# danielecook/seq-collection

Measured on AMD Instinct MI355X. Metric: Gbases/s parsed (fq-count), higher is better.
Workload: dtype u8; 1 GPU; synthetic 10 GB uncompressed 150 bp Illumina FASTQ per GPU, HBM-resident (BASELINE configs[1]; the N>1 lines of this bench hold 25 GB per GPU — `--bytes-per-gpu 25e9` at N=1 is their like-for-like anchor); bytes_per_gpu=10000000326, seed=20260101, exchange=none, flags=0

## Files before the change

seq-collection_amd/csrc/fq_scan_kernels.hpp:

```cpp
#pragma once
#include <hip/hip_runtime.h>
#include <stdint.h>

#include "scfq_hdrhash.hpp"

#ifndef SCFQ_ABLATE
#define SCFQ_ABLATE 0
#endif

namespace scfq {

constexpr int kTile = 4096;
constexpr int kWavesPerBlock = 4;
constexpr int kRing = 2;
constexpr int kPartialWords = 32;
constexpr uint32_t kMaxTilesPerRange = 960;

enum : int { W_NL = 0, W_GC = 1, W_N = 5, W_LEN = 9, W_STARTS = 13, W_FAT = 17, W_FPLUS = 21, W_BYTES = 25, W_LAST = 26 };

constexpr uint32_t F_QUAL_HIST = 1u, F_STRUCT = 2u;

constexpr int kHistRep = 4;
constexpr int kHistWords = 256 * 4 * kHistRep;
constexpr int kHistWaves = 2;
// ... 683 lines not shown
    }
    const uint32_t shl = (sh0 + cnt * 8u) & 31u;
    t_len += (64u - cnt - s_len) << shl;
    t_gc += (64u - popc64(WGC) - s_gc) << shl;
    t_nn += (64u - popc64(WNN) - s_nn) << shl;
  }

  st.p_len = t_len; st.p_gc = t_gc; st.p_nn = t_nn; st.p_crlf = t_crlf;
  if (STRUCT) { st.p_fat = t_fat; st.p_fpl = t_fpl; }
  if (++st.pending == 3) flush_pending(st);
  st.phase = (st.phase + total) & 3u;
  st.nl_total += total;
  st.prev_last = (int32_t)((uint32_t)__builtin_amdgcn_readlane((int)d[15], 63) >> 24);
}

struct ScanArgs {
  const uint8_t* base;
  uint64_t n;
  int32_t prev_byte;
  uint32_t tiles_per_range;
  uint64_t n_ranges;
  uint64_t* partials;
  uint32_t* hist_partials;
  const uint8_t* todo;
  const uint8_t* guess;
  uint32_t* hist_wg;
  uint8_t* guess_out;
  uint32_t guess_cap_tiles;
};

template <bool STRUCT, int HIST, int RING = kRing, bool NT = true, bool GUESS = false>
__global__ __launch_bounds__(HIST == 1 ? 64 * kHistWaves : HIST == 2 ? 64 * kQWaves : 64 * kWavesPerBlock, (HIST == 2 && !GUESS) ? SCFQ_QOCC : 1) void fq_scan_tiles(ScanArgs a) {
  constexpr int WAVES = HIST == 1 ? kHistWaves : HIST == 2 ? kQWaves : kWavesPerBlock;
  static_assert(RING >= 2 && RING <= 4, "ring depth");
  static_assert(!GUESS || (STRUCT && HIST == 0), "the guess pass is the K4 accounting without partials");
  extern __shared__ __attribute__((aligned(16))) uint8_t smem[];
  const int lane = threadIdx.x & 63;
  const uint32_t wave = (uint32_t)__builtin_amdgcn_readfirstlane((int)(threadIdx.x >> 6));
  uint8_t* ring = smem + (HIST == 2 ? kQWords * 4 : 0) + wave * (RING * kTile);
  const uint64_t range = (uint64_t)blockIdx.x * WAVES + wave;
  bool active = range < a.n_ranges;
  if (HIST == 1 && active && a.todo) active = (a.todo[range] != 0);
  if (HIST != 2 && !active) return;
  uint32_t* hist_lds = nullptr;
  if (HIST == 1) {
    hist_lds = reinterpret_cast<uint32_t*>(smem + WAVES * RING * kTile) + wave * kHistWords;
    for (int k = lane; k < kHistWords; k += 64) hist_lds[k] = 0;
  }
  if (HIST == 2) {
    hist_lds = reinterpret_cast<uint32_t*>(smem);
    if ((uint32_t)(uintptr_t)hist_lds & (kQWords * 4 - 1)) __builtin_trap();
    for (int k = threadIdx.x; k < kQWords; k += 64 * WAVES) hist_lds[k] = 0;
    __syncthreads();
  }
  if (active) {

  const uint64_t B = (uint64_t)(uintptr_t)a.base, E = B + a.n;
  const uint64_t A0 = B & ~(uint64_t)(kTile - 1);
// ... 96 lines not shown
      }
    }
  }
  if (GUESS) {
    if (lane == 0) a.guess_out[range] = (uint8_t)guessed;
    return;
  }

  flush_pending(st);
  uint64_t* out = a.partials + range * kPartialWords;
  auto sum4 = [&](const Acc16& acc) {
    const uint32_t c0 = wave_sum(acc.e & 0xFFFFu), c2 = wave_sum(acc.e >> 16);
    const uint32_t c1 = wave_sum(acc.o & 0xFFFFu), c3 = wave_sum(acc.o >> 16);
    return make_uint4(c0, c1, c2, c3);
  };
  auto store4 = [&](int w, uint64_t v0, uint64_t v1, uint64_t v2, uint64_t v3) {
    if (lane == 0) { out[w + 0] = v0; out[w + 1] = v1; out[w + 2] = v2; out[w + 3] = v3; }
  };
  const uint4 gc4 = sum4(st.gc), nn4 = sum4(st.nn), len4 = sum4(st.len), cr4 = sum4(st.crlf);
  store4(W_GC, gc4.x, gc4.y, gc4.z, gc4.w);
  store4(W_N, nn4.x, nn4.y, nn4.z, nn4.w);
  store4(W_LEN, (uint64_t)len4.x - cr4.x, (uint64_t)len4.y - cr4.y, (uint64_t)len4.z - cr4.z, (uint64_t)len4.w - cr4.w);
  if (STRUCT) {
    const uint4 a4 = sum4(st.fat), p4 = sum4(st.fplus);
    const uint64_t last_at = ((A0 + (uint64_t)t_end * kTile < E) ? A0 + (uint64_t)t_end * kTile : E) - 1;
    const uint32_t last_is_nl = (*reinterpret_cast<const uint8_t*>(last_at) == (uint8_t)'\n') ? 1u : 0u;
    const uint32_t nfol = st.nl_total - last_is_nl;
    const uint32_t first_is_start = (range_prev == '\n' || range_prev == -1) ? 1u : 0u;
    const uint4 s4 = make_uint4((nfol >> 2) + first_is_start, (nfol + 3u) >> 2, (nfol + 2u) >> 2, (nfol + 1u) >> 2);
    store4(W_STARTS, s4.x, s4.y, s4.z, s4.w);
    store4(W_FAT, a4.x, a4.y, a4.z, a4.w);
    store4(W_FPLUS, p4.x, p4.y, p4.z, p4.w);
  } else {
    store4(W_STARTS, 0, 0, 0, 0); store4(W_FAT, 0, 0, 0, 0); store4(W_FPLUS, 0, 0, 0, 0);
  }
  if (lane == 0) {
    out[W_NL] = st.nl_total;
    for (int k = W_BYTES; k < kPartialWords; ++k) out[k] = 0;
  }
  if (HIST == 2 && qcls < 4u) {
    const uint32_t crq = (qcls == 0) ? cr4.x : (qcls == 1) ? cr4.y : (qcls == 2) ? cr4.z : cr4.w;
    if (lane == 0 && crq) atomicSub(&hist_lds[13 * kQRep], crq);
    uint32_t bad = st.qbad;
    const uint32_t pivots = wave_sum(st.piv_cnt);
    const uint32_t pv = st.piv4 & 0xFFu;
    if (kQWindow && pivots && pv >= (uint32_t)kQBins) bad = 1u;
    if (lane == 0 && pivots) atomicAdd(&hist_lds[(pv & (uint32_t)(kQBins - 1)) * kQRep], 4u * pivots);
    {
      const uint4 lo4 = sum4(st.hot_lo), hi4 = sum4(st.hot_hi);
      const uint32_t tot[8] = {lo4.x, lo4.y, lo4.z, lo4.w, hi4.x, hi4.y, hi4.z, hi4.w};
#pragma unroll
      for (int k = 0; k < kHot; ++k) {
        const uint32_t v = ((k < 4 ? st.hotp[0] : st.hotp[1]) >> ((k & 3) * 8)) & 0xFFu;
        if (kQWindow && (uint32_t)k < st.n_hot && tot[k] && v >= (uint32_t)kQBins) bad = 1u;
// ... 18 lines not shown
  }
  if (HIST == 2) {
    __syncthreads();
    const uint32_t voided = kQWindow ? hist_lds[kQFlagWord] : 0u;
    for (uint32_t t = threadIdx.x; t < 256; t += 64 * WAVES) {
      uint32_t v = 0;
      if (t < (uint32_t)kQBins && !(kQWindow && t == 10u)) {
        const uint4* src = reinterpret_cast<const uint4*>(hist_lds + t * kQRep);
#pragma unroll
        for (int r = 0; r < kQRep / 4; ++r) { const uint4 q = src[r]; v += q.x + q.y + q.z + q.w; }
      }
      if (kQWindow && t == 255u && voided) v = kQPoison;
      a.hist_wg[(uint64_t)blockIdx.x * 256 + t] = v;
    }
  }
}


constexpr int kFoldThreads = 256;
constexpr int kFold1 = 128;

template <int T>
__device__ __forceinline__ uint32_t block_rotate_sum(const uint64_t* mine ,
                                                     uint32_t phase_in, uint64_t* lds_acc, uint32_t* lds_wave,
                                                     uint64_t (*rows)[W_BYTES + 1], int tid) {
  const int lane = tid & 63, w = tid >> 6;
  const uint32_t nl = (uint32_t)mine[W_NL];
  const uint32_t incl = wave_inclusive_scan(nl);
  if (lane == 63) lds_wave[w] = incl;
  __syncthreads();
  uint32_t before = 0;
#pragma unroll
  for (int k = 0; k < T / 64; ++k) before += (k < w) ? lds_wave[k] : 0u;
  const uint32_t phase = (phase_in + before + incl - nl) & 3u;
  rows[tid][W_NL] = mine[W_NL];
#pragma unroll
  for (int arr = W_GC; arr < W_BYTES; arr += 4) {
    uint64_t m0 = mine[arr], m1 = mine[arr + 1], m2 = mine[arr + 2], m3 = mine[arr + 3];
    const bool by1 = (phase & 1u) != 0, by2 = (phase & 2u) != 0;
    const uint64_t a0 = by1 ? m3 : m0, a1 = by1 ? m0 : m1, a2 = by1 ? m1 : m2, a3 = by1 ? m2 : m3;
    rows[tid][arr + 0] = by2 ? a2 : a0;
    rows[tid][arr + 1] = by2 ? a3 : a1;
    rows[tid][arr + 2] = by2 ? a0 : a2;
    rows[tid][arr + 3] = by2 ? a1 : a3;
  }
  __syncthreads();
  const int word = tid & 31, part = tid >> 5;
  if (word < W_BYTES) {
    uint64_t sum = 0;
    const int r0 = part * 32;
#pragma unroll 8
    for (int r = 0; r < 32; ++r) sum += rows[r0 + r][word];
    atomicAdd(reinterpret_cast<unsigned long long*>(&lds_acc[word]), (unsigned long long)sum);
  }
  __syncthreads();
  return phase;
}

__global__ __launch_bounds__(kFold1) void fq_fold_fused(const uint64_t* partials, uint64_t n_ranges, uint64_t* block_out,
                                                         uint32_t* ticket, uint64_t* state, int reset,
                                                         uint8_t* rel_phase, uint8_t* block_phase,
                                                         const uint8_t* base, uint64_t n) {
  __shared__ uint64_t acc[kPartialWords];
  __shared__ uint32_t wave_tot[kFold1 / 64];
  __shared__ uint64_t rows[kFold1][W_BYTES + 1];
  __shared__ uint32_t is_last;
  const int tid = threadIdx.x;
  const uint32_t n_blocks = gridDim.x;
  if (tid < kPartialWords) acc[tid] = 0;
  __syncthreads();
  {
    const uint64_t r = (uint64_t)blockIdx.x * kFold1 + tid;
    uint64_t mine[W_BYTES];
    const uint64_t* src = partials + r * kPartialWords;
#pragma unroll
    for (int k = 0; k < W_BYTES; ++k) mine[k] = (r < n_ranges) ? src[k] : 0;
    const uint32_t ph = block_rotate_sum<kFold1>(mine, 0u, acc, wave_tot, rows, tid);
    if (rel_phase && r < n_ranges) rel_phase[r] = (uint8_t)ph;
    if (tid < kPartialWords) block_out[(uint64_t)blockIdx.x * kPartialWords + tid] = (tid < W_BYTES) ? acc[tid] : 0;
  }
  asm volatile("s_waitcnt vmcnt(0)" ::: "memory");
  __syncthreads();
  if (tid == 0) {
    __builtin_amdgcn_fence(__ATOMIC_RELEASE, "agent");
    asm volatile("s_waitcnt vmcnt(0)" ::: "memory");
    const uint32_t t = __hip_atomic_fetch_add(ticket, 1u, __ATOMIC_RELAXED, __HIP_MEMORY_SCOPE_AGENT);
    is_last = (t == n_blocks - 1) ? 1u : 0u;
    if (is_last) {
      __builtin_amdgcn_fence(__ATOMIC_ACQUIRE, "agent");
      asm volatile("s_waitcnt vmcnt(0)" ::: "memory");
    }
  }
  __syncthreads();
  if (!is_last) return;
  uint32_t phase_in = reset ? 0u : ((uint32_t)state[W_NL] & 3u);
  uint64_t run = 0;
  const uint64_t old = (!reset && tid < W_BYTES) ? state[tid] : 0;
  for (uint32_t b0 = 0; b0 < n_blocks; b0 += kFold1) {
    if (tid < kPartialWords) acc[tid] = 0;
    __syncthreads();
    const uint32_t b = b0 + tid;
    uint64_t mine[W_BYTES];
    const uint64_t* src = block_out + (uint64_t)b * kPartialWords;
#pragma unroll
    for (int k = 0; k < W_BYTES; ++k) mine[k] = (b < n_blocks) ? src[k] : 0;
    const uint32_t ph = block_rotate_sum<kFold1>(mine, phase_in, acc, wave_tot, rows, tid);
    if (block_phase && b < n_blocks) block_phase[b] = (uint8_t)ph;
    if (tid < W_BYTES) run += acc[tid];
    phase_in = (phase_in + (uint32_t)acc[W_NL]) & 3u;
    __syncthreads();
  }
  if (tid < W_BYTES) state[tid] = old + run;
  if (tid == 0) {
    state[W_BYTES] = (reset ? 0 : state[W_BYTES]) + n;
    if (n) state[W_LAST] = base[n - 1]; else if (reset) state[W_LAST] = 0;
    *ticket = 0;
  }
}

__global__ __launch_bounds__(256) void fq_fold_hist(const uint32_t* hist_partials, const uint8_t* rel_phase,
                                                    const uint8_t* block_phase, uint64_t n_ranges, const uint8_t* todo,
                                                    unsigned long long* state_hist) {
  const uint32_t b = threadIdx.x;
  const uint64_t r0 = (uint64_t)blockIdx.x * kFold1;
  const uint64_t r1 = (r0 + kFold1 < n_ranges) ? r0 + kFold1 : n_ranges;
  const uint32_t bp = block_phase[blockIdx.x];
  uint64_t acc[4] = {0, 0, 0, 0};
  bool any = false;
  for (uint64_t r = r0; r < r1; ++r) {
    if (todo && !todo[r]) continue;
    any = true;
    const uint32_t ph = (bp + rel_phase[r]) & 3u;
// ... 640 lines not shown
```

seq-collection_amd/csrc/scfq_api.hip:

```cpp
#include "../../include/sc_fqcount.h"
#include "../../include/sc_fqcount_debug.h"
#include "fq_scan_kernels.hpp"
#include "scfq_bgzf.hpp"
#include "scfq_gzfast.hpp"
#include "scfq_pgz.hpp"
#include "bgzf_inflate_kernel.hpp"
#include "gz_inflate_kernels.hpp"
#include "scfq_arena.hpp"
#include "scfq_index_aux.hpp"

#include <fcntl.h>
#include <functional>
#include <sys/mman.h>
#include <sys/stat.h>
#include <unistd.h>
#include <zlib.h>

#include <algorithm>
#include <atomic>
#include <chrono>
#include <condition_variable>
#include <deque>
#include <cstdio>
#include <cstdlib>
#include <cstring>
#include <map>
#include <memory>
#include <mutex>
#include <string>
#include <thread>
#include <vector>

namespace {

thread_local char g_err[512] = "";

#define HIPCHK(call)                                                                          \
  do {                                                                                        \
    hipError_t e_ = (call);                                                                   \
    if (e_ != hipSuccess) {                                                                   \
      std::snprintf(g_err, sizeof g_err, "%s -> %s (%s:%d)", #call, hipGetErrorString(e_),    \
                    __FILE__, __LINE__);                                                      \
      if (std::getenv("SCFQ_VERBOSE")) std::fprintf(stderr, "scfq: %s\n", g_err);             \
      return SCFQ_EHIP;                                                                       \
    }                                                                                         \
  } while (0)

const std::chrono::steady_clock::time_point g_loaded = std::chrono::steady_clock::now();
inline int env_int_early(const char* name, int dflt) { const char* e = std::getenv(name); return e ? std::atoi(e) : dflt; }
inline bool trace_on() { static const bool v = std::getenv("SCFQ_VERBOSE") != nullptr; return v; }
struct StageLog { std::mutex mu; std::vector<std::pair<std::string, double>> v; };
inline StageLog& stage_log() { static StageLog* g = new StageLog; return *g; }
inline void trace(const char* what) {
  const double ms = std::chrono::duration<double, std::milli>(std::chrono::steady_clock::now() - g_loaded).count();
  {
    StageLog& g = stage_log();
    std::lock_guard<std::mutex> lk(g.mu);
    if (g.v.size() < 256) g.v.emplace_back(what, ms);
  }
  if (trace_on()) std::fprintf(stderr, "scfq t+%8.1f ms  %s\n", ms, what);
}
std::atomic<uint64_t> g_dev_bytes{0}, g_dev_high{0};
inline void note_dev_bytes(int64_t delta) {
  const uint64_t now = g_dev_bytes.fetch_add((uint64_t)delta) + (uint64_t)delta;
  uint64_t h = g_dev_high.load();
  while (now > h && !g_dev_high.compare_exchange_weak(h, now)) {}
}

constexpr uint64_t kDefaultChunk = 64ull << 20;
constexpr int kStateWords = SCFQ_PARTIAL_WORDS + SCFQ_HIST_WORDS + scfq::kExtWords;
constexpr int kExtAt = SCFQ_PARTIAL_WORDS + SCFQ_HIST_WORDS;

using scfq_arena::DevBuf;
using scfq_arena::SymPool;
struct GzSlot {
  SymPool sym;
  uint8_t* d_meta = nullptr;
  uint8_t* h_meta = nullptr;
};
constexpr int kGzMaxComp = 8, kGzMaxSlots = 6, kGzDecodeStreams = 3;
struct GzDevBuffers {
  DevBuf comp[kGzMaxComp];
  GzSlot slot[kGzMaxSlots];
  uint8_t* d_tables = nullptr;  uint64_t tables_cap = 0;
  uint8_t* h_tables = nullptr;  uint64_t htables_cap = 0;
  uint8_t* d_pmeta[kGzMaxSlots] = {};
// ... 49 lines not shown
  uint8_t* d_range_phase = nullptr;
  uint64_t cap_hist_ranges = 0;
  uint8_t* d_guess = nullptr;
  uint8_t* d_todo = nullptr;
  uint8_t* d_wg_ok = nullptr;
  uint32_t* d_hist_wg = nullptr;
  bool from_start = false;
  uint32_t last_tpr = 0;
  uint64_t last_ranges = 0;
  uint64_t* d_first_ord = nullptr;
  uint64_t cap_first_ord = 0;
  uint64_t* d_block_partials = nullptr;
  uint64_t cap_blocks = 0;
  uint64_t* d_state = nullptr;
  uint64_t* h_state = nullptr;
  std::vector<hipEvent_t> ev_pool;
  size_t ev_used = 0;
  std::vector<uint64_t> ev_bytes;
  std::vector<hipEvent_t> cp_pool;
  size_t cp_used = 0;
  uint32_t* d_ticket = nullptr;
  bool fresh = true;
  uint8_t* d_stage[2] = {nullptr, nullptr};
  uint8_t* d_comp[2] = {nullptr, nullptr};
  scfq_dinflate::Block* d_blk[2] = {nullptr, nullptr};
  scfq_dinflate::Block* h_blk[2] = {nullptr, nullptr};
  bool bgzf_warmed = false;
  hipEvent_t ev_piece[2] = {nullptr, nullptr};
  unsigned piece_it = 0;
  uint8_t* fg_stage[2] = {nullptr, nullptr};
  uint64_t fg_cap = 0;
  hipEvent_t ev_fg[2] = {nullptr, nullptr};
  unsigned fg_it = 0;
  bool fg_refused = false;
  uint8_t* d_inf[2] = {nullptr, nullptr};
  uint32_t* d_dstatus = nullptr;
// ... 77 lines not shown
  HIPCHK(hipDeviceGetAttribute(&n_cu, hipDeviceAttributeMultiprocessorCount, dev));
  c->n_cu = n_cu > 0 ? n_cu : 256;
  trace("  device attributes read");
  {
    int least = 0, greatest = 0;
    if (env_int_early("SCFQ_COMPUTE_PRIORITY", 0) && hipDeviceGetStreamPriorityRange(&least, &greatest) == hipSuccess && least != greatest)
      HIPCHK(hipStreamCreateWithPriority(&c->compute, hipStreamNonBlocking, greatest));
    else
      HIPCHK(hipStreamCreateWithFlags(&c->compute, hipStreamNonBlocking));
  }
  c->copy = c->compute;
  c->copy_is_alias = true;
  trace("  compute stream created");
  HIPCHK(hipMalloc(&c->d_state, kStateWords * sizeof(uint64_t) + 64));
  c->d_ticket = reinterpret_cast<uint32_t*>(c->d_state + kStateWords);
  HIPCHK(hipHostMalloc(&c->h_state, kStateWords * sizeof(uint64_t), hipHostMallocDefault));
  trace("  state words allocated (device + pinned)");
  HIPCHK(hipMemsetAsync(c->d_ticket, 0, sizeof(uint32_t), c->compute));
  for (int b = 0; b < 2; ++b) {
    HIPCHK(hipEventCreateWithFlags(&c->ev_copied[b], hipEventDisableTiming));
    HIPCHK(hipEventCreateWithFlags(&c->ev_scanned[b], hipEventDisableTiming));
  }
  *out = std::move(c);
  trace("context up");
  return SCFQ_OK;
}

int want_copy_stream(Ctx* c) {
  if (!c->copy_is_alias) return SCFQ_OK;
  hipStream_t st = nullptr;
  HIPCHK(hipStreamCreateWithFlags(&st, hipStreamNonBlocking));
  c->copy = st;
  c->copy_is_alias = false;
// ... 1 lines not shown
  return SCFQ_OK;
}

int ensure_partials(Ctx* c, uint64_t n_ranges, bool hist) {
  if (n_ranges > c->cap_ranges) {
    HIPCHK(hipStreamSynchronize(c->compute));
    if (c->d_partials) HIPCHK(hipFree(c->d_partials));
    c->d_partials = nullptr;
    uint64_t cap = std::max<uint64_t>(n_ranges + n_ranges / 4, 4096);
    HIPCHK(hipMalloc(&c->d_partials, cap * scfq::kPartialWords * sizeof(uint64_t)));
    c->cap_ranges = cap;
    if (c->d_block_partials) HIPCHK(hipFree(c->d_block_partials));
    c->d_block_partials = nullptr;
    c->cap_blocks = cap / scfq::kFold1 + 2;
    HIPCHK(hipMalloc(&c->d_block_partials, c->cap_blocks * scfq::kPartialWords * sizeof(uint64_t)));
  }
  if (hist && n_ranges > c->cap_hist_ranges) {
    HIPCHK(hipStreamSynchronize(c->compute));
    if (c->d_hist_partials) HIPCHK(hipFree(c->d_hist_partials));
    if (c->d_range_phase) HIPCHK(hipFree(c->d_range_phase));
    if (c->d_guess) HIPCHK(hipFree(c->d_guess));
    if (c->d_hist_wg) HIPCHK(hipFree(c->d_hist_wg));
    c->d_hist_partials = nullptr;
    c->d_range_phase = nullptr;
    c->d_guess = nullptr;
    c->d_hist_wg = nullptr;
    uint64_t cap = std::max<uint64_t>(n_ranges + n_ranges / 4, 4096);
    HIPCHK(hipMalloc(&c->d_hist_partials, cap * 1024 * sizeof(uint32_t)));
    HIPCHK(hipMalloc(&c->d_range_phase, 2 * cap));
    HIPCHK(hipMalloc(&c->d_guess, 3 * cap));
// ... 48 lines not shown
  if (!GUESS)
    std::snprintf(g_last_scan, sizeof g_last_scan, "fq_scan_tiles<%s, %d, %d, %s, %s> tiles_per_range=%u", S ? "true" : "false", H, RING, NT ? "true" : "false",
                  GUESS ? "true" : "false", a.tiles_per_range);
  constexpr int waves = (H == 1) ? scfq::kHistWaves : (H == 2) ? scfq::kQWaves : scfq::kWavesPerBlock;
  unsigned lds = waves * RING * scfq::kTile;
  if (H == 1) lds += waves * scfq::kHistWords * sizeof(uint32_t);
  if (H == 2) lds += scfq::kQWords * sizeof(uint32_t);
  (void)blocks;
  const unsigned grid = (unsigned)((a.n_ranges + waves - 1) / waves);
  hipLaunchKernelGGL((scfq::fq_scan_tiles<S, H, RING, NT, GUESS>), dim3(grid), dim3(64 * waves), lds, st, a);
}

int env_int(const char* name, int dflt) {
  const char* e = std::getenv(name);
  return e ? std::atoi(e) : dflt;
}

int scan_async(Ctx* c, const uint8_t* dptr, uint64_t n, int prev_byte, uint32_t flags, bool timing) {
  if (n == 0) return SCFQ_OK;
  const bool hist = flags & SCFQ_QUAL_HIST, strct = flags & SCFQ_STRUCT_CHECK;
  const uint64_t B = (uint64_t)(uintptr_t)dptr, A0 = B & ~(uint64_t)(scfq::kTile - 1);
  const uint64_t NT = (B + n - A0 + scfq::kTile - 1) / scfq::kTile;
  if (NT >= (1ull << 32)) { std::snprintf(g_err, sizeof g_err, "a single scan launch covers at most 16 TiB"); return SCFQ_EARG; }
  const uint32_t tpr = pick_tiles_per_range(c, NT);
  const uint64_t n_ranges = (NT + tpr - 1) / tpr;
  int rc = ensure_partials(c, n_ranges, hist);
  if (rc) return rc;
  c->last_tpr = tpr;
  c->last_ranges = n_ranges;
  scfq::ScanArgs a;
  a.base = dptr;
  a.n = n;
  a.prev_byte = prev_byte;
  a.tiles_per_range = tpr;
  a.n_ranges = n_ranges;
  a.partials = c->d_partials;
  a.hist_partials = c->d_hist_partials;
  const unsigned blocks = (unsigned)((n_ranges + scfq::kWavesPerBlock - 1) / scfq::kWavesPerBlock);
  hipEvent_t ev[3] = {nullptr, nullptr, nullptr};
  if (timing) {
    while (c->ev_pool.size() < c->ev_used + 3) { hipEvent_t e; HIPCHK(hipEventCreate(&e)); c->ev_pool.push_back(e); }
    for (int k = 0; k < 3; ++k) ev[k] = c->ev_pool[c->ev_used + k];
    c->ev_used += 3;
    c->ev_bytes.push_back(n);
    HIPCHK(hipEventRecord(ev[0], c->compute));
  }
  static const int hist_mode_env = [] { const char* e = std::getenv("SCFQ_HIST_MODE"); return !e ? 0 : (e[0] == 'e' ? 1 : 2); }();
  const bool spec = hist && (hist_mode_env ? hist_mode_env == 2 : !(flags & SCFQ_HIST_EXACT));
  a.todo = nullptr;
  a.guess = c->d_guess;
  a.hist_wg = c->d_hist_wg;
  a.guess_out = c->d_guess;
// ... 4 lines not shown
    else launch_scan<false, 2, 2, true>(a, blocks, c->compute);
  }
  else if (hist && strct) launch_scan<true, 1, 2, true>(a, blocks, c->compute);
  else if (hist) launch_scan<false, 1, 2, true>(a, blocks, c->compute);
  else if (strct) launch_scan<true, 0, 2, true>(a, blocks, c->compute);
  else {
    static const int ring = env_int("SCFQ_RING", 2), nt = env_int("SCFQ_NT", 1);
    if (ring == 2 && nt) launch_scan<false, 0, 2, true>(a, blocks, c->compute);
    else if (ring == 2) launch_scan<false, 0, 2, false>(a, blocks, c->compute);
    else if (ring == 4 && nt) launch_scan<false, 0, 4, true>(a, blocks, c->compute);
    else if (ring == 4) launch_scan<false, 0, 4, false>(a, blocks, c->compute);
    else if (nt) launch_scan<false, 0, 3, true>(a, blocks, c->compute);
    else launch_scan<false, 0, 3, false>(a, blocks, c->compute);
  }
  HIPCHK(hipGetLastError());
  if (timing) HIPCHK(hipEventRecord(ev[1], c->compute));
  {
    const uint64_t n_blocks = (n_ranges + scfq::kFold1 - 1) / scfq::kFold1;
    uint8_t* rel_phase = hist ? c->d_range_phase : nullptr;
    uint8_t* block_phase = hist ? c->d_range_phase + c->cap_hist_ranges : nullptr;
    if (hist && c->fresh)
      HIPCHK(hipMemsetAsync(c->d_state + SCFQ_PARTIAL_WORDS, 0, (SCFQ_HIST_WORDS + scfq::kExtWords) * sizeof(uint64_t), c->compute));
    hipLaunchKernelGGL(scfq::fq_fold_fused, dim3((unsigned)n_blocks), dim3(scfq::kFold1), 0, c->compute, c->d_partials,
                       n_ranges, c->d_block_partials, c->d_ticket, c->d_state, c->fresh ? 1 : 0, rel_phase, block_phase,
                       dptr, n);
    HIPCHK(hipGetLastError());
    c->fresh = false;
    unsigned long long* state_hist = (unsigned long long*)(c->d_state + SCFQ_PARTIAL_WORDS);
    if (spec) {
      uint64_t* ext = c->d_state + kExtAt;
      const uint64_t n_wg = (n_ranges + scfq::kQWaves - 1) / scfq::kQWaves;
      hipLaunchKernelGGL(scfq::fq_hist_verify, dim3((unsigned)((n_wg + 255) / 256)), dim3(256), 0, c->compute, c->d_guess, rel_phase, block_phase, n_ranges,
                         c->from_start ? 0 : -1, ext, c->d_todo, c->d_wg_ok, c->d_hist_wg);
      HIPCHK(hipGetLastError());
      a.todo = c->d_todo;
      if (strct) launch_scan<true, 1, 2, true>(a, blocks, c->compute);
      else launch_scan<false, 1, 2, true>(a, blocks, c->compute);
      HIPCHK(hipGetLastError());
      hipLaunchKernelGGL(scfq::fq_fold_hist, dim3((unsigned)n_blocks), dim3(256), 0, c->compute, c->d_hist_partials,
                         rel_phase, block_phase, n_ranges, c->d_todo, state_hist);
// ... 7 lines not shown
    }
  }
  if (timing) HIPCHK(hipEventRecord(ev[2], c->compute));
  return SCFQ_OK;
}

int begin_session(Ctx* c, bool from_start) {
  ++c->n_sessions;
  c->from_start = from_start;
  c->timing = scfq_timing{};
  c->timing.struct_size = sizeof(scfq_timing);
  c->ev_used = 0;
  c->cp_used = 0;
  c->ev_bytes.clear();
  c->fresh = true;
  return SCFQ_OK;
}

int end_session(Ctx* c, bool hist, scfq_partial* out, uint64_t* hist_out) {
  const size_t words = hist ? kStateWords : SCFQ_PARTIAL_WORDS;
  if (c->fresh) {
    std::memset(c->h_state, 0, words * sizeof(uint64_t));
  } else {
    HIPCHK(hipMemcpyAsync(c->h_state, c->d_state, words * sizeof(uint64_t), hipMemcpyDeviceToHost, c->compute));
    HIPCHK(hipStreamSynchronize(c->compute));
  }
  for (size_t k = 0; k + 2 < c->ev_used + 0 && k < c->ev_used; k += 3) {
    float ms1 = 0, ms2 = 0;
    HIPCHK(hipEventElapsedTime(&ms1, c->ev_pool[k], c->ev_pool[k + 1]));
    HIPCHK(hipEventElapsedTime(&ms2, c->ev_pool[k + 1], c->ev_pool[k + 2]));
    c->timing.scan_kernel_ms += ms1;
    c->timing.fold_kernel_ms += ms2;
    c->timing.scan_bytes += c->ev_bytes[k / 3];
    c->timing.scan_launches += 1;
  }
  for (size_t k = 0; k + 1 < c->cp_used; k += 2) {
    float ms = 0;
    HIPCHK(hipEventElapsedTime(&ms, c->cp_pool[k], c->cp_pool[k + 1]));
    c->timing.h2d_ms += ms;
  }
  trace("session folded");
  std::memcpy(out, c->h_state, sizeof(scfq_partial));
  out->hist_class = 0;
  g_hist_stats[0] = g_hist_stats[1] = 0;
  if (hist) {
    const uint64_t h1 = c->h_state[kExtAt + scfq::kExtH];
    out->hist_class = h1 ? (((h1 - 1) + 3) & 3u) + 1 : 0;
    g_hist_stats[0] = c->h_state[kExtAt + scfq::kExtFast];
    g_hist_stats[1] = c->h_state[kExtAt + scfq::kExtRedo];
  }
// ... 1352 lines not shown
  std::lock_guard<std::mutex> lk(g_mu);
  for (auto& kv : g_ctx)
   for (auto& up : kv.second) {
    Ctx* c = up.get();
    (void)hipSetDevice(c->dev);
    if (c->compute) (void)hipStreamSynchronize(c->compute);
    if (c->copy) (void)hipStreamSynchronize(c->copy);
    if (c->h_pin[0]) (void)hipHostFree(c->h_pin[0]);
    for (int b = 0; b < 2; ++b) {
      if (c->d_stage[b]) (void)hipFree(c->d_stage[b]);
      if (c->ev_copied[b]) (void)hipEventDestroy(c->ev_copied[b]);
      if (c->ev_scanned[b]) (void)hipEventDestroy(c->ev_scanned[b]);
    }
    if (c->d_partials) (void)hipFree(c->d_partials);
    if (c->d_block_partials) (void)hipFree(c->d_block_partials);
    if (c->d_hist_partials) (void)hipFree(c->d_hist_partials);
    if (c->d_range_phase) (void)hipFree(c->d_range_phase);
    if (c->d_guess) (void)hipFree(c->d_guess);
    if (c->d_hist_wg) (void)hipFree(c->d_hist_wg);
    if (c->d_first_ord) (void)hipFree(c->d_first_ord);
    for (int b = 0; b < 2; ++b) {
      if (c->d_comp[b]) (void)hipFree(c->d_comp[b]);
      if (c->d_inf[b]) (void)hipFree(c->d_inf[b]);
      if (c->d_blk[b]) (void)hipFree(c->d_blk[b]);
      if (c->h_blk[b]) (void)hipHostFree(c->h_blk[b]);
      if (c->ev_piece[b]) (void)hipEventDestroy(c->ev_piece[b]);
      if (c->ev_fg[b]) (void)hipEventDestroy(c->ev_fg[b]);
      if (c->fg_stage[b]) (void)hipFree(c->fg_stage[b]);
    }
    note_dev_bytes(-(int64_t)(2 * c->fg_cap));
// ... 580 lines not shown
  Ctx* c = nullptr;
  SessionLock sl;
  int rc = get_ctx(&c, sl);
  if (rc) return rc;
  rc = begin_session(c, false);
  if (rc) return rc;
  if (n) {
    const uint64_t chunks = (n + 255) / 256;
    rc = ensure_partials(c, chunks, false);
    if (rc) return rc;
    hipLaunchKernelGGL(scfq::fq_scan_simple, dim3((unsigned)((chunks + 255) / 256)), dim3(256), 0, c->compute,
                       static_cast<const uint8_t*>(dptr), n, prev_byte, chunks, c->d_partials);
    HIPCHK(hipGetLastError());
    const uint64_t n_blocks = (chunks + scfq::kFold1 - 1) / scfq::kFold1;
    hipLaunchKernelGGL(scfq::fq_fold_fused, dim3((unsigned)n_blocks), dim3(scfq::kFold1), 0, c->compute, c->d_partials,
                       chunks, c->d_block_partials, c->d_ticket, c->d_state, 1, (uint8_t*)nullptr, (uint8_t*)nullptr,
                       static_cast<const uint8_t*>(dptr), n);
    HIPCHK(hipGetLastError());
    c->fresh = false;
  }
  return end_session(c, false, out, nullptr);
}

}
```

Before: 2706 Gbases/s.

## Fuse partial fold into scan kernel via last-arriver tickets and mapped host state

Folds the per-range partials inside the scan kernel. The last workgroup of each 128-range group reduces that group, and the last group then does the global fold, so the separate fold kernel launch is gone in the non-histogram path. The result is written straight into a device-mapped pinned host mirror, which removes the device-to-host copy at session end. Partials are now stored with one lane per word instead of serial lane-0 stores. This adds ticket atomics, LDS reuse of the tile ring, and ticket-reset handling after errors.

```diff
diff --git a/seq-collection_amd/csrc/fq_scan_kernels.hpp b/seq-collection_amd/csrc/fq_scan_kernels.hpp
--- a/seq-collection_amd/csrc/fq_scan_kernels.hpp
+++ b/seq-collection_amd/csrc/fq_scan_kernels.hpp
@@ -721,6 +721,151 @@
   st.prev_last = (int32_t)((uint32_t)__builtin_amdgcn_readlane((int)d[15], 63) >> 24);
 }
 
+
+constexpr int kFold1 = 128;
+
+struct FoldLds {
+  uint64_t acc[kPartialWords];
+  uint32_t wave_tot[kFold1 / 64];
+  uint32_t flag;
+  uint32_t pad_;
+  uint64_t rows[kFold1][W_BYTES + 1];
+};
+static_assert(sizeof(FoldLds) <= (size_t)kWavesPerBlock * kRing * kTile, "the fold works inside the scan's tile ring");
+
+template <int T>
+__device__ __forceinline__ uint32_t block_rotate_sum(const uint64_t* mine ,
+                                                     uint32_t phase_in, FoldLds& s, int tid) {
+  const int lane = tid & 63, w = tid >> 6;
+  const bool in = tid < T;
+  const uint32_t nl = in ? (uint32_t)mine[W_NL] : 0u;
+  uint32_t incl = 0;
+  if (in) {
+    incl = wave_inclusive_scan(nl);
+    if (lane == 63) s.wave_tot[w] = incl;
+  }
+  __syncthreads();
+  uint32_t phase = 0;
+  if (in) {
+    uint32_t before = 0;
+#pragma unroll
+    for (int k = 0; k < T / 64; ++k) before += (k < w) ? s.wave_tot[k] : 0u;
+    phase = (phase_in + before + incl - nl) & 3u;
+    s.rows[tid][W_NL] = mine[W_NL];
+#pragma unroll
+    for (int arr = W_GC; arr < W_BYTES; arr += 4) {
+      uint64_t m0 = mine[arr], m1 = mine[arr + 1], m2 = mine[arr + 2], m3 = mine[arr + 3];
+      const bool by1 = (phase & 1u) != 0, by2 = (phase & 2u) != 0;
+      const uint64_t a0 = by1 ? m3 : m0, a1 = by1 ? m0 : m1, a2 = by1 ? m1 : m2, a3 = by1 ? m2 : m3;
+      s.rows[tid][arr + 0] = by2 ? a2 : a0;
+      s.rows[tid][arr + 1] = by2 ? a3 : a1;
+      s.rows[tid][arr + 2] = by2 ? a0 : a2;
+      s.rows[tid][arr + 3] = by2 ? a1 : a3;
+    }
+  }
+  __syncthreads();
+  const int word = tid & 31, part = tid >> 5;
+  if (in && word < W_BYTES) {
+    uint64_t sum = 0;
+    const int r0 = part * 32;
+#pragma unroll 8
+    for (int r = 0; r < 32; ++r) sum += s.rows[r0 + r][word];
+    atomicAdd(reinterpret_cast<unsigned long long*>(&s.acc[word]), (unsigned long long)sum);
+  }
+  __syncthreads();
+  return phase;
+}
+
+__device__ __forceinline__ bool fold_last_arriver(FoldLds& s, uint32_t* counter, uint32_t members, int tid) {
+  asm volatile("s_waitcnt vmcnt(0)" ::: "memory");
+  __syncthreads();
+  if (tid == 0) {
+    __builtin_amdgcn_fence(__ATOMIC_RELEASE, "agent");
+    asm volatile("s_waitcnt vmcnt(0)" ::: "memory");
+    const uint32_t t = atomicInc(counter, members - 1u);
+    const uint32_t last = (t == members - 1u) ? 1u : 0u;
+    s.flag = last;
+    if (last) {
+      __builtin_amdgcn_fence(__ATOMIC_ACQUIRE, "agent");
+      asm volatile("s_waitcnt vmcnt(0)" ::: "memory");
+    }
+  }
+  __syncthreads();
+  return s.flag != 0u;
+}
+
+__device__ __forceinline__ uint32_t fold_level1(FoldLds& s, const uint64_t* partials, uint64_t n_ranges, uint32_t group,
+                                                uint64_t* block_out, int tid) {
+  if (tid < kPartialWords) s.acc[tid] = 0;
+  __syncthreads();
+  const uint64_t r = (uint64_t)group * kFold1 + tid;
+  const bool have = tid < kFold1 && r < n_ranges;
+  uint64_t mine[W_BYTES];
+  const uint64_t* src = partials + (have ? r : (uint64_t)group * kFold1) * kPartialWords;
+#pragma unroll
+  for (int k = 0; k < W_BYTES; ++k) mine[k] = src[k];
+#pragma unroll
+  for (int k = 0; k < W_BYTES; ++k) mine[k] = have ? mine[k] : 0;
+  const uint32_t ph = block_rotate_sum<kFold1>(mine, 0u, s, tid);
+  if (tid < kPartialWords) block_out[(uint64_t)group * kPartialWords + tid] = (tid < W_BYTES) ? s.acc[tid] : 0;
+  return ph;
+}
+
+struct FoldOut {
+  uint64_t* state;
+  uint64_t* host_state;
+  uint64_t* ticks;
+  uint64_t* host_ticks;
+  int reset;
+  const uint8_t* base;
+  uint64_t n;
+};
+
+__device__ __forceinline__ void fold_level2(FoldLds& s, const uint64_t* block_out, uint32_t n_blocks, const FoldOut& o,
+                                            uint8_t* block_phase, int tid) {
+  const uint64_t t0 = wall_clock64();
+  uint32_t phase_in = o.reset ? 0u : ((uint32_t)o.state[W_NL] & 3u);
+  uint64_t run = 0;
+  const uint64_t old = (!o.reset && tid < W_BYTES) ? o.state[tid] : 0;
+  for (uint32_t b0 = 0; b0 < n_blocks; b0 += kFold1) {
+    if (tid < kPartialWords) s.acc[tid] = 0;
+    __syncthreads();
+    const uint32_t b = b0 + tid;
+    const bool have = tid < kFold1 && b < n_blocks;
+    uint64_t mine[W_BYTES];
+    const uint64_t* src = block_out + (uint64_t)(have ? b : 0u) * kPartialWords;
+#pragma unroll
+    for (int k = 0; k < W_BYTES; ++k) mine[k] = src[k];
+#pragma unroll
+    for (int k = 0; k < W_BYTES; ++k) mine[k] = have ? mine[k] : 0;
+    const uint32_t ph = block_rotate_sum<kFold1>(mine, phase_in, s, tid);
+    if (block_phase && have) block_phase[b] = (uint8_t)ph;
+    if (tid < W_BYTES) run += s.acc[tid];
+    phase_in = (phase_in + (uint32_t)s.acc[W_NL]) & 3u;
+    __syncthreads();
+  }
+  if (tid < W_BYTES) {
+    const uint64_t v = old + run;
+    o.state[tid] = v;
+    if (o.host_state) o.host_state[tid] = v;
+  }
+  if (tid == 0) {
+    const uint64_t bytes = (o.reset ? 0 : o.state[W_BYTES]) + o.n;
+    const uint64_t last = o.n ? (uint64_t)o.base[o.n - 1] : (o.reset ? 0 : o.state[W_LAST]);
+    o.state[W_BYTES] = bytes;
+    o.state[W_LAST] = last;
+    if (o.host_state) { o.host_state[W_BYTES] = bytes; o.host_state[W_LAST] = last; }
+  }
+  if (o.host_state && tid > W_LAST && tid < kPartialWords) o.host_state[tid] = 0;
+  if (tid == 0) {
+    const uint64_t before = o.reset ? 0 : *o.ticks;
+    asm volatile("s_waitcnt vmcnt(0)" ::: "memory");
+    const uint64_t t = before + (wall_clock64() - t0);
+    *o.ticks = t;
+    if (o.host_ticks) *o.host_ticks = t;
+  }
+}
+
 struct ScanArgs {
   const uint8_t* base;
   uint64_t n;
@@ -734,6 +879,10 @@
   uint32_t* hist_wg;
   uint8_t* guess_out;
   uint32_t guess_cap_tiles;
+  uint64_t* block_out;
+  uint32_t* group_tickets;
+  uint32_t* ticket;
+  FoldOut fold;
 };
 
 template <bool STRUCT, int HIST, int RING = kRing, bool NT = true, bool GUESS = false>
@@ -748,7 +897,8 @@
   const uint64_t range = (uint64_t)blockIdx.x * WAVES + wave;
   bool active = range < a.n_ranges;
   if (HIST == 1 && active && a.todo) active = (a.todo[range] != 0);
-  if (HIST != 2 && !active) return;
+  constexpr bool FOLD = (HIST == 0 && !GUESS);
+  if (HIST != 2 && !FOLD && !active) return;
   uint32_t* hist_lds = nullptr;
   if (HIST == 1) {
     hist_lds = reinterpret_cast<uint32_t*>(smem + WAVES * RING * kTile) + wave * kHistWords;
@@ -875,8 +1025,9 @@
     const uint32_t c1 = wave_sum(acc.o & 0xFFFFu), c3 = wave_sum(acc.o >> 16);
     return make_uint4(c0, c1, c2, c3);
   };
+  uint64_t pw = 0;
   auto store4 = [&](int w, uint64_t v0, uint64_t v1, uint64_t v2, uint64_t v3) {
-    if (lane == 0) { out[w + 0] = v0; out[w + 1] = v1; out[w + 2] = v2; out[w + 3] = v3; }
+    pw = (lane == w) ? v0 : (lane == w + 1) ? v1 : (lane == w + 2) ? v2 : (lane == w + 3) ? v3 : pw;
   };
   const uint4 gc4 = sum4(st.gc), nn4 = sum4(st.nn), len4 = sum4(st.len), cr4 = sum4(st.crlf);
   store4(W_GC, gc4.x, gc4.y, gc4.z, gc4.w);
@@ -892,13 +1043,9 @@
     store4(W_STARTS, s4.x, s4.y, s4.z, s4.w);
     store4(W_FAT, a4.x, a4.y, a4.z, a4.w);
     store4(W_FPLUS, p4.x, p4.y, p4.z, p4.w);
-  } else {
-    store4(W_STARTS, 0, 0, 0, 0); store4(W_FAT, 0, 0, 0, 0); store4(W_FPLUS, 0, 0, 0, 0);
-  }
-  if (lane == 0) {
-    out[W_NL] = st.nl_total;
-    for (int k = W_BYTES; k < kPartialWords; ++k) out[k] = 0;
-  }
+  }
+  if (lane == W_NL) pw = st.nl_total;
+  if (lane < kPartialWords) out[lane] = pw;
   if (HIST == 2 && qcls < 4u) {
     const uint32_t crq = (qcls == 0) ? cr4.x : (qcls == 1) ? cr4.y : (qcls == 2) ? cr4.z : cr4.w;
     if (lane == 0 && crq) atomicSub(&hist_lds[13 * kQRep], crq);
@@ -947,108 +1094,30 @@
       a.hist_wg[(uint64_t)blockIdx.x * 256 + t] = v;
     }
   }
-}
-
-
-constexpr int kFoldThreads = 256;
-constexpr int kFold1 = 128;
-
-template <int T>
-__device__ __forceinline__ uint32_t block_rotate_sum(const uint64_t* mine ,
-                                                     uint32_t phase_in, uint64_t* lds_acc, uint32_t* lds_wave,
-                                                     uint64_t (*rows)[W_BYTES + 1], int tid) {
-  const int lane = tid & 63, w = tid >> 6;
-  const uint32_t nl = (uint32_t)mine[W_NL];
-  const uint32_t incl = wave_inclusive_scan(nl);
-  if (lane == 63) lds_wave[w] = incl;
-  __syncthreads();
-  uint32_t before = 0;
-#pragma unroll
-  for (int k = 0; k < T / 64; ++k) before += (k < w) ? lds_wave[k] : 0u;
-  const uint32_t phase = (phase_in + before + incl - nl) & 3u;
-  rows[tid][W_NL] = mine[W_NL];
-#pragma unroll
-  for (int arr = W_GC; arr < W_BYTES; arr += 4) {
-    uint64_t m0 = mine[arr], m1 = mine[arr + 1], m2 = mine[arr + 2], m3 = mine[arr + 3];
-    const bool by1 = (phase & 1u) != 0, by2 = (phase & 2u) != 0;
-    const uint64_t a0 = by1 ? m3 : m0, a1 = by1 ? m0 : m1, a2 = by1 ? m1 : m2, a3 = by1 ? m2 : m3;
-    rows[tid][arr + 0] = by2 ? a2 : a0;
-    rows[tid][arr + 1] = by2 ? a3 : a1;
-    rows[tid][arr + 2] = by2 ? a0 : a2;
-    rows[tid][arr + 3] = by2 ? a1 : a3;
-  }
-  __syncthreads();
-  const int word = tid & 31, part = tid >> 5;
-  if (word < W_BYTES) {
-    uint64_t sum = 0;
-    const int r0 = part * 32;
-#pragma unroll 8
-    for (int r = 0; r < 32; ++r) sum += rows[r0 + r][word];
-    atomicAdd(reinterpret_cast<unsigned long long*>(&lds_acc[word]), (unsigned long long)sum);
-  }
-  __syncthreads();
-  return phase;
+  if (FOLD) {
+    if (!a.block_out) return;
+    FoldLds& s = *reinterpret_cast<FoldLds*>(smem);
+    const int tid = threadIdx.x;
+    constexpr uint32_t kWgPerGroup = kFold1 / kWavesPerBlock;
+    const uint32_t n_groups = (uint32_t)((a.n_ranges + kFold1 - 1) / kFold1);
+    const uint32_t group = blockIdx.x / kWgPerGroup;
+    const uint32_t members = (group + 1 < n_groups) ? kWgPerGroup : gridDim.x - group * kWgPerGroup;
+    if (!fold_last_arriver(s, a.group_tickets + group, members, tid)) return;
+    fold_level1(s, a.partials, a.n_ranges, group, a.block_out, tid);
+    if (!fold_last_arriver(s, a.ticket, n_groups, tid)) return;
+    fold_level2(s, a.block_out, n_groups, a.fold, nullptr, tid);
+  }
 }
 
 __global__ __launch_bounds__(kFold1) void fq_fold_fused(const uint64_t* partials, uint64_t n_ranges, uint64_t* block_out,
-                                                         uint32_t* ticket, uint64_t* state, int reset,
-                                                         uint8_t* rel_phase, uint8_t* block_phase,
-                                                         const uint8_t* base, uint64_t n) {
-  __shared__ uint64_t acc[kPartialWords];
-  __shared__ uint32_t wave_tot[kFold1 / 64];
-  __shared__ uint64_t rows[kFold1][W_BYTES + 1];
-  __shared__ uint32_t is_last;
+                                                         uint32_t* ticket, FoldOut o, uint8_t* rel_phase, uint8_t* block_phase) {
+  __shared__ FoldLds s;
   const int tid = threadIdx.x;
-  const uint32_t n_blocks = gridDim.x;
-  if (tid < kPartialWords) acc[tid] = 0;
-  __syncthreads();
-  {
-    const uint64_t r = (uint64_t)blockIdx.x * kFold1 + tid;
-    uint64_t mine[W_BYTES];
-    const uint64_t* src = partials + r * kPartialWords;
-#pragma unroll
-    for (int k = 0; k < W_BYTES; ++k) mine[k] = (r < n_ranges) ? src[k] : 0;
-    const uint32_t ph = block_rotate_sum<kFold1>(mine, 0u, acc, wave_tot, rows, tid);
-    if (rel_phase && r < n_ranges) rel_phase[r] = (uint8_t)ph;
-    if (tid < kPartialWords) block_out[(uint64_t)blockIdx.x * kPartialWords + tid] = (tid < W_BYTES) ? acc[tid] : 0;
-  }
-  asm volatile("s_waitcnt vmcnt(0)" ::: "memory");
-  __syncthreads();
-  if (tid == 0) {
-    __builtin_amdgcn_fence(__ATOMIC_RELEASE, "agent");
-    asm volatile("s_waitcnt vmcnt(0)" ::: "memory");
-    const uint32_t t = __hip_atomic_fetch_add(ticket, 1u, __ATOMIC_RELAXED, __HIP_MEMORY_SCOPE_AGENT);
-    is_last = (t == n_blocks - 1) ? 1u : 0u;
-    if (is_last) {
-      __builtin_amdgcn_fence(__ATOMIC_ACQUIRE, "agent");
-      asm volatile("s_waitcnt vmcnt(0)" ::: "memory");
-    }
-  }
-  __syncthreads();
-  if (!is_last) return;
-  uint32_t phase_in = reset ? 0u : ((uint32_t)state[W_NL] & 3u);
-  uint64_t run = 0;
-  const uint64_t old = (!reset && tid < W_BYTES) ? state[tid] : 0;
-  for (uint32_t b0 = 0; b0 < n_blocks; b0 += kFold1) {
-    if (tid < kPartialWords) acc[tid] = 0;
-    __syncthreads();
-    const uint32_t b = b0 + tid;
-    uint64_t mine[W_BYTES];
-    const uint64_t* src = block_out + (uint64_t)b * kPartialWords;
-#pragma unroll
-    for (int k = 0; k < W_BYTES; ++k) mine[k] = (b < n_blocks) ? src[k] : 0;
-    const uint32_t ph = block_rotate_sum<kFold1>(mine, phase_in, acc, wave_tot, rows, tid);
-    if (block_phase && b < n_blocks) block_phase[b] = (uint8_t)ph;
-    if (tid < W_BYTES) run += acc[tid];
-    phase_in = (phase_in + (uint32_t)acc[W_NL]) & 3u;
-    __syncthreads();
-  }
-  if (tid < W_BYTES) state[tid] = old + run;
-  if (tid == 0) {
-    state[W_BYTES] = (reset ? 0 : state[W_BYTES]) + n;
-    if (n) state[W_LAST] = base[n - 1]; else if (reset) state[W_LAST] = 0;
-    *ticket = 0;
-  }
+  const uint32_t ph = fold_level1(s, partials, n_ranges, blockIdx.x, block_out, tid);
+  const uint64_t r = (uint64_t)blockIdx.x * kFold1 + tid;
+  if (rel_phase && r < n_ranges) rel_phase[r] = (uint8_t)ph;
+  if (!fold_last_arriver(s, ticket, gridDim.x, tid)) return;
+  fold_level2(s, block_out, gridDim.x, o, block_phase, tid);
 }
 
 __global__ __launch_bounds__(256) void fq_fold_hist(const uint32_t* hist_partials, const uint8_t* rel_phase,
diff --git a/seq-collection_amd/csrc/scfq_api.hip b/seq-collection_amd/csrc/scfq_api.hip
--- a/seq-collection_amd/csrc/scfq_api.hip
+++ b/seq-collection_amd/csrc/scfq_api.hip
@@ -34,6 +34,7 @@
 namespace {
 
 thread_local char g_err[512] = "";
+std::atomic<uint32_t> g_hip_errors{0};
 
 #define HIPCHK(call)                                                                          \
   do {                                                                                        \
@@ -42,6 +43,7 @@
       std::snprintf(g_err, sizeof g_err, "%s -> %s (%s:%d)", #call, hipGetErrorString(e_),    \
                     __FILE__, __LINE__);                                                      \
       if (std::getenv("SCFQ_VERBOSE")) std::fprintf(stderr, "scfq: %s\n", g_err);             \
+      g_hip_errors.fetch_add(1);                                                              \
       return SCFQ_EHIP;                                                                       \
     }                                                                                         \
   } while (0)
@@ -70,6 +72,7 @@
 constexpr uint64_t kDefaultChunk = 64ull << 20;
 constexpr int kStateWords = SCFQ_PARTIAL_WORDS + SCFQ_HIST_WORDS + scfq::kExtWords;
 constexpr int kExtAt = SCFQ_PARTIAL_WORDS + SCFQ_HIST_WORDS;
+constexpr uint64_t kEvFolded = 1ull << 63;
 
 using scfq_arena::DevBuf;
 using scfq_arena::SymPool;
@@ -149,12 +152,19 @@
   uint64_t cap_blocks = 0;
   uint64_t* d_state = nullptr;
   uint64_t* h_state = nullptr;
+  uint64_t* h_state_dev = nullptr;
+  bool fold_in_scan = true;
+  bool folded_apart = false;
+  double tick_ms = 1e-5;
+  uint32_t* d_group_tickets = nullptr;
+  uint32_t hip_errors_seen = 0;
   std::vector<hipEvent_t> ev_pool;
   size_t ev_used = 0;
   std::vector<uint64_t> ev_bytes;
   std::vector<hipEvent_t> cp_pool;
   size_t cp_used = 0;
   uint32_t* d_ticket = nullptr;
+  uint64_t* d_fold_ticks = nullptr;
   bool fresh = true;
   uint8_t* d_stage[2] = {nullptr, nullptr};
   uint8_t* d_comp[2] = {nullptr, nullptr};
@@ -262,9 +272,21 @@
   trace("  compute stream created");
   HIPCHK(hipMalloc(&c->d_state, kStateWords * sizeof(uint64_t) + 64));
   c->d_ticket = reinterpret_cast<uint32_t*>(c->d_state + kStateWords);
-  HIPCHK(hipHostMalloc(&c->h_state, kStateWords * sizeof(uint64_t), hipHostMallocDefault));
+  c->d_fold_ticks = c->d_state + kStateWords + 1;
+  HIPCHK(hipHostMalloc(&c->h_state, (kStateWords + 1) * sizeof(uint64_t), hipHostMallocDefault));
+  std::memset(c->h_state, 0, (kStateWords + 1) * sizeof(uint64_t));
+  {
+    void* dp = nullptr;
+    if (env_int_early("SCFQ_HOST_MIRROR", 1) && hipHostGetDevicePointer(&dp, c->h_state, 0) == hipSuccess && dp) c->h_state_dev = static_cast<uint64_t*>(dp);
+    else { (void)hipGetLastError(); trace("  no device address for the pinned state mirror: the result is copied"); }
+    int khz = 0;
+    if (hipDeviceGetAttribute(&khz, hipDeviceAttributeWallClockRate, dev) == hipSuccess && khz > 0) c->tick_ms = 1.0 / (double)khz;
+    else (void)hipGetLastError();
+    c->fold_in_scan = env_int_early("SCFQ_FOLD_IN_SCAN", 1) != 0;
+  }
   trace("  state words allocated (device + pinned)");
-  HIPCHK(hipMemsetAsync(c->d_ticket, 0, sizeof(uint32_t), c->compute));
+  HIPCHK(hipMemsetAsync(c->d_state + kStateWords, 0, 64, c->compute));
+  c->hip_errors_seen = g_hip_errors.load();
   for (int b = 0; b < 2; ++b) {
     HIPCHK(hipEventCreateWithFlags(&c->ev_copied[b], hipEventDisableTiming));
     HIPCHK(hipEventCreateWithFlags(&c->ev_scanned[b], hipEventDisableTiming));
@@ -296,6 +318,15 @@
     c->d_block_partials = nullptr;
     c->cap_blocks = cap / scfq::kFold1 + 2;
     HIPCHK(hipMalloc(&c->d_block_partials, c->cap_blocks * scfq::kPartialWords * sizeof(uint64_t)));
+    if (c->d_group_tickets) HIPCHK(hipFree(c->d_group_tickets));
+    c->d_group_tickets = nullptr;
+    HIPCHK(hipMalloc(&c->d_group_tickets, c->cap_blocks * sizeof(uint32_t)));
+    HIPCHK(hipMemsetAsync(c->d_group_tickets, 0, c->cap_blocks * sizeof(uint32_t), c->compute));
+  }
+  if (c->hip_errors_seen != g_hip_errors.load()) {
+    c->hip_errors_seen = g_hip_errors.load();
+    HIPCHK(hipMemsetAsync(c->d_group_tickets, 0, c->cap_blocks * sizeof(uint32_t), c->compute));
+    HIPCHK(hipMemsetAsync(c->d_ticket, 0, sizeof(uint32_t), c->compute));
   }
   if (hist && n_ranges > c->cap_hist_ranges) {
     HIPCHK(hipStreamSynchronize(c->compute));
@@ -374,6 +405,18 @@
 int env_int(const char* name, int dflt) {
   const char* e = std::getenv(name);
   return e ? std::atoi(e) : dflt;
+}
+
+scfq::FoldOut fold_out(Ctx* c, const uint8_t* base, uint64_t n) {
+  scfq::FoldOut o;
+  o.state = c->d_state;
+  o.host_state = c->h_state_dev;
+  o.ticks = c->d_fold_ticks;
+  o.host_ticks = c->h_state_dev ? c->h_state_dev + kStateWords : nullptr;
+  o.reset = c->fresh ? 1 : 0;
+  o.base = base;
+  o.n = n;
+  return o;
 }
 
 int scan_async(Ctx* c, const uint8_t* dptr, uint64_t n, int prev_byte, uint32_t flags, bool timing) {
@@ -396,6 +439,11 @@
   a.n_ranges = n_ranges;
   a.partials = c->d_partials;
   a.hist_partials = c->d_hist_partials;
+  const bool fold_in_scan = !hist && c->fold_in_scan;
+  a.block_out = fold_in_scan ? c->d_block_partials : nullptr;
+  a.group_tickets = c->d_group_tickets;
+  a.ticket = c->d_ticket;
+  a.fold = fold_out(c, dptr, n);
   const unsigned blocks = (unsigned)((n_ranges + scfq::kWavesPerBlock - 1) / scfq::kWavesPerBlock);
   hipEvent_t ev[3] = {nullptr, nullptr, nullptr};
   if (timing) {
@@ -430,6 +478,12 @@
     else launch_scan<false, 0, 3, false>(a, blocks, c->compute);
   }
   HIPCHK(hipGetLastError());
+  if (fold_in_scan) {
+    c->fresh = false;
+    if (timing) { HIPCHK(hipEventRecord(ev[2], c->compute)); c->ev_bytes.back() |= kEvFolded; }
+    return SCFQ_OK;
+  }
+  c->folded_apart = true;
   if (timing) HIPCHK(hipEventRecord(ev[1], c->compute));
   {
     const uint64_t n_blocks = (n_ranges + scfq::kFold1 - 1) / scfq::kFold1;
@@ -438,8 +492,7 @@
     if (hist && c->fresh)
       HIPCHK(hipMemsetAsync(c->d_state + SCFQ_PARTIAL_WORDS, 0, (SCFQ_HIST_WORDS + scfq::kExtWords) * sizeof(uint64_t), c->compute));
     hipLaunchKernelGGL(scfq::fq_fold_fused, dim3((unsigned)n_blocks), dim3(scfq::kFold1), 0, c->compute, c->d_partials,
-                       n_ranges, c->d_block_partials, c->d_ticket, c->d_state, c->fresh ? 1 : 0, rel_phase, block_phase,
-                       dptr, n);
+                       n_ranges, c->d_block_partials, c->d_ticket, a.fold, rel_phase, block_phase);
     HIPCHK(hipGetLastError());
     c->fresh = false;
     unsigned long long* state_hist = (unsigned long long*)(c->d_state + SCFQ_PARTIAL_WORDS);
@@ -477,6 +530,7 @@
   c->cp_used = 0;
   c->ev_bytes.clear();
   c->fresh = true;
+  c->folded_apart = false;
   return SCFQ_OK;
 }
 
@@ -485,18 +539,29 @@
   if (c->fresh) {
     std::memset(c->h_state, 0, words * sizeof(uint64_t));
   } else {
-    HIPCHK(hipMemcpyAsync(c->h_state, c->d_state, words * sizeof(uint64_t), hipMemcpyDeviceToHost, c->compute));
+    if (!c->h_state_dev) {
+      HIPCHK(hipMemcpyAsync(c->h_state, c->d_state, words * sizeof(uint64_t), hipMemcpyDeviceToHost, c->compute));
+      HIPCHK(hipMemcpyAsync(c->h_state + kStateWords, c->d_fold_ticks, sizeof(uint64_t), hipMemcpyDeviceToHost, c->compute));
+    } else if (hist) {
+      HIPCHK(hipMemcpyAsync(c->h_state + SCFQ_PARTIAL_WORDS, c->d_state + SCFQ_PARTIAL_WORDS, (words - SCFQ_PARTIAL_WORDS) * sizeof(uint64_t),
+                            hipMemcpyDeviceToHost, c->compute));
+    }
     HIPCHK(hipStreamSynchronize(c->compute));
   }
   for (size_t k = 0; k + 2 < c->ev_used + 0 && k < c->ev_used; k += 3) {
     float ms1 = 0, ms2 = 0;
-    HIPCHK(hipEventElapsedTime(&ms1, c->ev_pool[k], c->ev_pool[k + 1]));
-    HIPCHK(hipEventElapsedTime(&ms2, c->ev_pool[k + 1], c->ev_pool[k + 2]));
+    if (c->ev_bytes[k / 3] & kEvFolded) {
+      HIPCHK(hipEventElapsedTime(&ms1, c->ev_pool[k], c->ev_pool[k + 2]));
+    } else {
+      HIPCHK(hipEventElapsedTime(&ms1, c->ev_pool[k], c->ev_pool[k + 1]));
+      HIPCHK(hipEventElapsedTime(&ms2, c->ev_pool[k + 1], c->ev_pool[k + 2]));
+    }
     c->timing.scan_kernel_ms += ms1;
     c->timing.fold_kernel_ms += ms2;
-    c->timing.scan_bytes += c->ev_bytes[k / 3];
+    c->timing.scan_bytes += c->ev_bytes[k / 3] & ~kEvFolded;
     c->timing.scan_launches += 1;
   }
+  if (!c->fresh && !c->folded_apart && c->ev_used) c->timing.fold_kernel_ms = (double)c->h_state[kStateWords] * c->tick_ms;
   for (size_t k = 0; k + 1 < c->cp_used; k += 2) {
     float ms = 0;
     HIPCHK(hipEventElapsedTime(&ms, c->cp_pool[k], c->cp_pool[k + 1]));
@@ -1879,6 +1944,7 @@
     }
     if (c->d_partials) (void)hipFree(c->d_partials);
     if (c->d_block_partials) (void)hipFree(c->d_block_partials);
+    if (c->d_group_tickets) (void)hipFree(c->d_group_tickets);
     if (c->d_hist_partials) (void)hipFree(c->d_hist_partials);
     if (c->d_range_phase) (void)hipFree(c->d_range_phase);
     if (c->d_guess) (void)hipFree(c->d_guess);
@@ -2489,8 +2555,8 @@
     HIPCHK(hipGetLastError());
     const uint64_t n_blocks = (chunks + scfq::kFold1 - 1) / scfq::kFold1;
     hipLaunchKernelGGL(scfq::fq_fold_fused, dim3((unsigned)n_blocks), dim3(scfq::kFold1), 0, c->compute, c->d_partials,
-                       chunks, c->d_block_partials, c->d_ticket, c->d_state, 1, (uint8_t*)nullptr, (uint8_t*)nullptr,
-                       static_cast<const uint8_t*>(dptr), n);
+                       chunks, c->d_block_partials, c->d_ticket, fold_out(c, static_cast<const uint8_t*>(dptr), n),
+                       (uint8_t*)nullptr, (uint8_t*)nullptr);
     HIPCHK(hipGetLastError());
     c->fresh = false;
   }
```

Result: slower. 2347 Gbases/s (-13.3%).
